# shg8/3DGS.cpp

Measured on NVIDIA B200. Metric: frames/sec, higher is better.
Workload: dtype f32

## Files before the change

### 3dgs.cpp_b200/csrc/gsb_api.cu

```cuda
#include <math.h>
#include <stdio.h>
#include <stdlib.h>
#include <string.h>

#include <algorithm>
#include <new>
#include <thread>
#include <vector>

#include "gsb_ctx.cuh"

using namespace gsb;

namespace {
thread_local std::string g_create_error;
}

namespace gsb {

int fail(gsb_ctx* c, int code, const char* what, cudaError_t e) {
    if (c) {
        c->err = what;
        if (e != cudaSuccess) {
            c->err += ": ";
// ... 108 lines not shown
    SortParams sa{};
    sa.keys[0] = ctx->dkeys[0];
    sa.keys[1] = ctx->dkeys[1];
    sa.vals[0] = ctx->dvals[0];
    sa.vals[1] = ctx->dvals[1];
    sa.key_bytes = 4;
    sa.d_m = &ctx->ctl->num_visible;
    sa.m_hint = fp.nv_q;
    sa.key_bits = 32;
    sa.status = ctx->sort_status;
    sa.status_tiles = ctx->sort_status_tiles;
    sa.d_epoch = &ctx->ctl->epoch;
    sa.epoch_base = 0;
    sa.sc = &ctx->ctl->sort_depth;
    sa.num_sms = ctx->num_sms;
    sa.events = nullptr;
    sa.ranges = nullptr;
    sa.discard_sorted_keys = true;
    uint32_t depth_passes = 0;
    CK(launch_sort(sa, &depth_passes, stream));
    const int fin_a = depth_passes & 1;
    if (events) CK(cudaEventRecord(ctx->ev[2], stream));

    EmitParams ep{};
    ep.sorted_cid = ctx->dvals[fin_a];
    ep.nv_hint = fp.nv_q;
    ep.tiles_x = fp.bins_x;
    ep.coarse_shift = fp.cs;
    ep.keys = ctx->keys[0];
    ep.vals = ctx->vals[0];
    ep.capacity = (uint32_t)ctx->capacity;
// ... 22 lines not shown
    SortParams sp{};
    sp.keys[0] = ctx->keys[0];
    sp.keys[1] = ctx->keys[1];
    sp.vals[0] = ctx->vals[0];
    sp.vals[1] = ctx->vals[1];
    sp.key_bytes = 4;
    sp.d_m = &ctx->ctl->num_instances;
    sp.m_hint = fp.m_q;
    sp.key_bits = bits_for(fp.bins);
    sp.status = ctx->sort_status;
    sp.status_tiles = ctx->sort_status_tiles;
    sp.d_epoch = &ctx->ctl->epoch;
    sp.epoch_base = 4;
    sp.sc = &ctx->ctl->sort_tile;
    sp.num_sms = ctx->num_sms;
    sp.events = events ? ctx->ev_sort : nullptr;
    sp.ranges = ctx->ranges;
    sp.discard_sorted_keys = !ctx->debug && fp.cs == 0;
    sp.range_key_mask = fp.cs ? 0xffffu : 0u;
    uint32_t passes = 0;
    CK(launch_sort(sp, &passes, stream));
    if (events) CK(cudaEventRecord(ctx->ev[4], stream));
    if (passes == 0) CK(launch_ranges_single_tile(sp.d_m, ctx->ranges, stream));
    if (events) CK(cudaEventRecord(ctx->ev[5], stream));
    if (depth_passes != fp.depth_passes || passes != fp.passes) return fail(ctx, GSB_ERR_CUDA, "internal: pass count mismatch");
    return GSB_OK;
}

int launch_middle_graph(gsb_ctx* ctx, const FramePlan& fp, cudaStream_t stream) {
    MiddleKey key;
    key.tiles_x = fp.tiles_x;
// ... 146 lines not shown
    bp.variant = ctx->blend_variant;
    bp.stats = ctx->debug ? 2 : (ctx->timers ? 1 : 0);
    bp.one = 1.0f;
    bp.ctl = ctx->ctl;
    if (band_aux) {
        bp.aux = reinterpret_cast<float2*>(static_cast<unsigned char*>(band_aux) + (size_t)(b0 - fp.rb) * GSB_TILE * aux_pitch);
        bp.aux_pitch = aux_pitch;
    }
    CK(launch_blend(bp, stream));
    return GSB_OK;
}

int enqueue_tail(gsb_ctx* ctx, const FramePlan& fp, cudaStream_t stream) {
    if (ctx->timers) CK(cudaEventRecord(ctx->ev[6], stream));
    CK(cudaMemcpyAsync(ctx->ctl_host, ctx->ctl, offsetof(Control, sort_depth), cudaMemcpyDeviceToHost, stream));
    CK(cudaEventRecord(ctx->ev_done, stream));
    ctx->frame_pending = true;
    ctx->have_frame = true;
    ctx->frame_debug = ctx->debug;
    ctx->frame_timers = ctx->timers;
    ctx->last_w = fp.W;
    ctx->last_h = fp.H;
    ctx->last_tiles_x = fp.tiles_x;
    ctx->last_tiles_y = fp.tiles_y;
    ctx->last_passes = fp.passes;
    ctx->last_depth_passes = fp.depth_passes;
    ctx->last_final = (uint32_t)fp.fin;
    return GSB_OK;
}

// ... 71 lines not shown
        gsb_destroy(ctx);
        return GSB_ERR_NO_DEVICE;
    }
    ctx->num_sms = prop.multiProcessorCount;
    if (const char* v = getenv("GSB_BLEND_VARIANT")) ctx->blend_variant = atoi(v) == 1 ? 1 : 2;
    if (const char* v = getenv("GSB_HOST_DIRECT")) ctx->host_direct = atoi(v) != 0;
    if (const char* v = getenv("GSB_COARSE_SHIFT")) ctx->coarse_shift = (uint32_t)std::min(2, std::max(1, atoi(v)));
    if ((e = sort_prepare()) != cudaSuccess) return bail("sort_prepare", e);
    if ((e = cudaStreamCreateWithFlags(&ctx->stream, cudaStreamNonBlocking)) != cudaSuccess) return bail("cudaStreamCreate", e);
    if ((e = dev_alloc(&ctx->ctl, 1)) != cudaSuccess) return bail("cudaMalloc", e);
    if ((e = cudaMemset(ctx->ctl, 0, sizeof(Control))) != cudaSuccess) return bail("cudaMemset", e);
    if ((e = cudaDeviceSynchronize()) != cudaSuccess) return bail("cudaDeviceSynchronize", e);
    if ((e = cudaMallocHost(reinterpret_cast<void**>(&ctx->ctl_host), sizeof(Control))) != cudaSuccess) return bail("cudaMallocHost", e);
    memset(ctx->ctl_host, 0, sizeof(Control));
    for (auto& ev : ctx->ev)
        if ((e = cudaEventCreate(&ev)) != cudaSuccess) return bail("cudaEventCreate", e);
    for (auto& ev : ctx->ev_sort)
        if ((e = cudaEventCreate(&ev)) != cudaSuccess) return bail("cudaEventCreate", e);
    if ((e = cudaEventCreateWithFlags(&ctx->ev_done, cudaEventDisableTiming)) != cudaSuccess) return bail("cudaEventCreate", e);
    *out = ctx;
    return GSB_OK;
}

void gsb_destroy(gsb_ctx* ctx) {
    if (!ctx) return;
    cudaSetDevice(ctx->device);
    if (ctx->stream) cudaStreamSynchronize(ctx->stream);
    cudaDeviceSynchronize();
    drop_graphs(ctx);
    shard_destroy(ctx);
    dev_free(ctx->dbg_offsets);
    dev_free(ctx->pos_op);
// ... 6 lines not shown
    dev_free(ctx->emit_status);
    dev_free(ctx->recs);
    dev_free(ctx->dkeys[0]);
    dev_free(ctx->dkeys[1]);
    dev_free(ctx->dvals[0]);
    dev_free(ctx->dvals[1]);
    free_arena(ctx);
    dev_free(ctx->ranges);
    if (ctx->fb) cudaFree(ctx->fb);
    if (ctx->aux_fb) cudaFree(ctx->aux_fb);
    dev_free(ctx->dbg_tiles);
    dev_free(ctx->dbg_aabb);
    dev_free(ctx->dbg_keys_unsorted);
    dev_free(ctx->dbg_vals_unsorted);
    for (auto& ev : ctx->ev)
        if (ev) cudaEventDestroy(ev);
    for (auto& ev : ctx->ev_sort)
        if (ev) cudaEventDestroy(ev);
    if (ctx->ev_done) cudaEventDestroy(ctx->ev_done);
    if (ctx->stream) cudaStreamDestroy(ctx->stream);
    delete ctx;
}

int gsb_scene_upload(gsb_ctx* ctx, const float* vertices, uint64_t n, gsb_memory mem) {
    if (!ctx) return GSB_ERR_INVALID;
    if (n && !vertices) return fail(ctx, GSB_ERR_INVALID, "null vertices");
    if (n >= (1ull << 30)) return fail(ctx, GSB_ERR_INVALID, "scene limited to 2^30 - 1 Gaussians");
    CK(cudaSetDevice(ctx->device));
    CK(cudaStreamSynchronize(ctx->stream));
    ctx->frame_pending = false;
    ctx->have_frame = false;
    dev_free(ctx->pos_op);
// ... 292 lines not shown
    out->sort_passes = ctx->last_passes;
    out->sort_depth_passes = ctx->last_depth_passes;
    out->regrow_count = ctx->regrow_count;
    if (ctx->frame_timers) {
        float ms = 0.f;
        CK(cudaEventElapsedTime(&ms, ctx->ev[0], ctx->ev[1]));
        out->preprocess_ms = ms;
        CK(cudaEventElapsedTime(&ms, ctx->ev[1], ctx->ev[2]));
        out->sort_depth_ms = ms;
        CK(cudaEventElapsedTime(&ms, ctx->ev[2], ctx->ev[3]));
        out->preprocess_sort_ms = ms;
        CK(cudaEventElapsedTime(&ms, ctx->ev[3], ctx->ev[4]));
        out->sort_tile_ms = ms;
        out->sort_ms = out->sort_depth_ms + out->sort_tile_ms;
        if (ctx->last_passes) {
            CK(cudaEventElapsedTime(&ms, ctx->ev[3], ctx->ev_sort[0]));
            out->sort_hist_ms = ms;
            for (uint32_t p = 0; p < ctx->last_passes && p < 8; p++) {
                CK(cudaEventElapsedTime(&ms, ctx->ev_sort[p], ctx->ev_sort[p + 1]));
                out->sort_pass_ms[p] = ms;
            }
        }
        CK(cudaEventElapsedTime(&ms, ctx->ev[4], ctx->ev[5]));
        out->tile_boundary_ms = ms;
        CK(cudaEventElapsedTime(&ms, ctx->ev[5], ctx->ev[6]));
        out->render_ms = ms;
        CK(cudaEventElapsedTime(&ms, ctx->ev[0], ctx->ev[6]));
        out->frame_ms = ms;
        if (ctx->shard) {
            CK(cudaEventElapsedTime(&ms, ctx->ev[5], ctx->ev[7]));
            out->shard_blend_ms = ms;
            CK(cudaEventElapsedTime(&ms, ctx->ev[7], ctx->ev[6]));
            out->shard_wait_ms = ms;
        }
    }
    if (c->overflow || c->overflow_sticky) {
// ... 179 lines not shown
    SortParams sp{};
    sp.keys[0] = keys;
    sp.keys[1] = keys_tmp;
    sp.key_bytes = key_bytes;
    sp.vals[0] = vals;
    sp.vals[1] = vals_tmp;
    sp.d_m = &ctx->ctl->num_instances;
    sp.m_hint = m32;
    sp.key_bits = key_bits;
    sp.status = status;
    sp.status_tiles = tiles;
    sp.d_epoch = nullptr;
    sp.epoch_base = 8;
    sp.sc = &ctx->ctl->sort_tile;
    sp.num_sms = ctx->num_sms;
    sp.events = nullptr;
    sp.ranges = nullptr;
    uint32_t passes = 0;
    if (e == cudaSuccess) e = launch_sort(sp, &passes, s);
    if (e == cudaSuccess && (passes & 1)) {
        e = cudaMemcpyAsync(keys, keys_tmp, m * (size_t)key_bytes, cudaMemcpyDeviceToDevice, s);
        if (e == cudaSuccess) e = cudaMemcpyAsync(vals, vals_tmp, m * 4, cudaMemcpyDeviceToDevice, s);
    }
    if (e == cudaSuccess) e = cudaStreamSynchronize(s);
    cudaFree(status);
    if (e != cudaSuccess) return fail(ctx, GSB_ERR_CUDA, what, e);
    return GSB_OK;
}

int gsb_sort_pairs(gsb_ctx* ctx, uint64_t* keys, uint32_t* vals, uint64_t* keys_tmp, uint32_t* vals_tmp, uint64_t m,
                   uint32_t key_bits, void* stream) {
// ... 10 lines not shown
```

### 3dgs.cpp_b200/csrc/gsb_ctx.cuh

```cuda
#pragma once
#include <algorithm>
#include <string>

#include "gsb_internal.cuh"

namespace gsb {
struct ShardState;
}
using gsb::Control;

struct MiddleKey {
    uint32_t tiles_x = 0, num_tiles = 0, nv_q = 0, m_q = 0, cull = 0, tag = 0, cs = 0;
    uint64_t alloc_gen = 0;
    bool operator==(const MiddleKey& o) const {
        return tiles_x == o.tiles_x && num_tiles == o.num_tiles && nv_q == o.nv_q && m_q == o.m_q && cull == o.cull && tag == o.tag &&
               cs == o.cs && alloc_gen == o.alloc_gen;
    }
};
struct MiddleGraph {
    MiddleKey key;
    cudaGraphExec_t exec = nullptr;
    uint64_t last_use = 0;
};

// ... 26 lines not shown
    uint32_t sort_status_tiles = 0;
    uint32_t epoch = 8;
    uint2* ranges = nullptr;
    uint32_t ranges_tiles = 0;
    void* fb = nullptr;
    size_t fb_bytes = 0;
    void* aux_fb = nullptr;
    size_t aux_fb_bytes = 0;

    int mode = GSB_MODE_EXACT;
    bool debug = false;
    bool timers = true;
    int tile_cull = 0;
    uint32_t coarse_shift = 2;
    cudaEvent_t ev[8] = {};
    cudaEvent_t ev_sort[9] = {};
    cudaEvent_t ev_done = nullptr;
    bool frame_pending = false;
    bool have_frame = false;
    bool frame_debug = false;
    bool frame_timers = false;
    bool host_direct = true;
    int blend_variant = 2;
    bool use_graph = true;
    uint64_t alloc_gen = 0;
    uint64_t graph_clock = 0;
    uint32_t frames_since_epoch_clear = 0;
    MiddleGraph graphs[4] = {};
    uint32_t m_hint = 0;
    uint32_t nv_hint = 0;
    uint32_t regrow_count = 0;
// ... 63 lines not shown
```

### 3dgs.cpp_b200/csrc/gsb_internal.cuh

```cuda
#pragma once
#include <cuda_runtime.h>
#include <stdint.h>

#include <string>

#include "gs_b200.h"

#define GSB_TILE 16
#define GSB_REC_F4 4
#define GSB_MAX_SHARDS 8

namespace gsb {

struct SortCtl {
    uint32_t ticket[8];
    uint32_t hist[8][256];
};

struct Control {
    uint32_t project_ticket;
    uint32_t emit_ticket;
    uint32_t num_visible;
    uint32_t num_instances;
    uint32_t overflow;
    uint32_t overflow_sticky;
    uint32_t epoch;
    uint32_t pad0;
    unsigned long long instances_total;
    unsigned long long blend_consumed;
    unsigned long long candidates_total;
// ... 52 lines not shown
cudaError_t launch_emit(const EmitParams& p, cudaStream_t s);

struct SortParams {
    void* keys[2];
    uint32_t* vals[2];
    int key_bytes;
    const uint32_t* d_m;
    uint32_t m_hint;
    uint32_t key_bits;
    unsigned long long* status;
    uint32_t status_tiles;
    const uint32_t* d_epoch;
    uint32_t epoch_base;
    SortCtl* sc;
    int num_sms;
    cudaEvent_t* events;
    uint2* ranges;
    uint32_t range_key_mask;
    bool discard_sorted_keys;
};
cudaError_t launch_sort(const SortParams& p, uint32_t* passes, cudaStream_t s);
uint32_t sort_tile_items();

cudaError_t launch_frame_init(Control* ctl, uint32_t* project_status, uint32_t project_chunks, unsigned long long* emit_status,
                              uint32_t emit_chunks, uint2* ranges, uint32_t num_tiles, cudaStream_t s, uint32_t* extra_words = nullptr,
                              uint32_t num_extra_words = 0);
cudaError_t sort_prepare();
cudaError_t launch_ranges_single_tile(const uint32_t* d_m, uint2* ranges, cudaStream_t s);

struct BlendParams {
    const float4* recs;
// ... 24 lines not shown
```

### 3dgs.cpp_b200/csrc/gsb_sort.cu

```cuda
#include "gsb_internal.cuh"
#include "gsb_tma.cuh"

namespace gsb {

namespace {

#ifndef GSB_SORT_MATCH_ATOMIC
#define GSB_SORT_MATCH_ATOMIC 1
#endif
constexpr int SORT_IPT = 16;
#ifndef GSB_SORT_THREADS
#define GSB_SORT_THREADS 256
#endif
constexpr int SORT_THREADS = GSB_SORT_THREADS;
constexpr int SORT_TILE = SORT_THREADS * SORT_IPT;
constexpr int SORT_WARPS = SORT_THREADS / 32;
constexpr int RADIX = 256;
constexpr unsigned FULL = 0xffffffffu;

#ifndef GSB_HIST_CTAS
#define GSB_HIST_CTAS 3
#endif
constexpr int HIST_THREADS = 512;
constexpr int HIST_IPT = 8;
constexpr int HIST_TILE = HIST_THREADS * HIST_IPT;

constexpr uint32_t LB_AGG = 1u << 30;
constexpr uint32_t LB_PREFIX = 2u << 30;
constexpr uint32_t LB_COUNT = (1u << 30) - 1u;
#ifndef GSB_LB_WINDOW
#define GSB_LB_WINDOW 8
#endif
constexpr int LB_WINDOW = GSB_LB_WINDOW;

__device__ __forceinline__ unsigned long long ld_volatile(const unsigned long long* p) {
    return *reinterpret_cast<const volatile unsigned long long*>(p);
}
__device__ __forceinline__ void st_volatile(unsigned long long* p, unsigned long long v) {
    *reinterpret_cast<volatile unsigned long long*>(p) = v;
}

template <typename KeyT>
__device__ __forceinline__ KeyT key_max();
template <>
__device__ __forceinline__ uint32_t key_max<uint32_t>() {
    return 0xffffffffu;
}
template <>
__device__ __forceinline__ unsigned long long key_max<unsigned long long>() {
    return ~0ull;
}

template <typename KeyT, int P>
__global__ void __launch_bounds__(HIST_THREADS) k_sort_hist(const KeyT* __restrict__ keys, const uint32_t* __restrict__ d_m,
                                                            SortCtl* sc) {
    __shared__ uint32_t s_hist[P][RADIX];
    const int tid = threadIdx.x;
    for (int k = tid; k < P * RADIX; k += HIST_THREADS) (&s_hist[0][0])[k] = 0;
    __syncthreads();
    const uint32_t m = *d_m;
    const uint32_t num_tiles = (m + HIST_TILE - 1) / HIST_TILE;
    for (uint32_t tile = blockIdx.x; tile < num_tiles; tile += gridDim.x) {
        const uint32_t base = tile * HIST_TILE;
        KeyT k[HIST_IPT];
#pragma unroll
        for (int it = 0; it < HIST_IPT; it++) {
            const uint32_t idx = base + it * HIST_THREADS + tid;
            k[it] = idx < m ? __ldg(keys + idx) : key_max<KeyT>();
        }
#pragma unroll
        for (int it = 0; it < HIST_IPT; it++) {
            const uint32_t idx = base + it * HIST_THREADS + tid;
            const bool valid = idx < m;
#pragma unroll
            for (int p = 0; p < P; p++) {
                const uint32_t d = (uint32_t)(k[it] >> (8 * p)) & 255u;
                const uint32_t d0 = __shfl_sync(FULL, d, 0);
                const unsigned same = __ballot_sync(FULL, valid && d == d0);
                if ((threadIdx.x & 31) == 0) {
                    if (same) atomicAdd(&s_hist[p][d0], (uint32_t)__popc(same));
                } else if (valid && d != d0) {
                    atomicAdd(&s_hist[p][d], 1u);
                }
            }
        }
    }
    __syncthreads();
    for (int k = tid; k < P * RADIX; k += HIST_THREADS) {
        const uint32_t c = (&s_hist[0][0])[k];
        if (c) atomicAdd(&sc->hist[0][0] + k, c);
    }
}

template <typename KeyT>
constexpr bool kMatchAtomic = GSB_SORT_MATCH_ATOMIC && sizeof(KeyT) == 4;
template <typename KeyT>
struct PassSmem {
    KeyT keys[2][SORT_TILE];
    uint32_t vals[2][SORT_TILE];
    uint32_t whist[SORT_WARPS][RADIX];
    uint32_t match[kMatchAtomic<KeyT> ? SORT_WARPS : 1][RADIX];
    uint32_t bin_start[RADIX];
    int32_t out_base[RADIX];
    uint32_t gexcl[RADIX];
    uint32_t warp_sums[SORT_WARPS];
    unsigned long long mbar[2];
// ... 27 lines not shown
        if (lane >= o) incl += t;
    }
    if (lane == 31) warp_sums[warp] = incl;
    __syncthreads();
    uint32_t before = 0;
#pragma unroll
    for (int w = 0; w < NW; w++) {
        const uint32_t s = warp_sums[w];
        if (w < warp) before += s;
    }
    __syncthreads();
    return before + incl - v;
}

template <typename KeyT>
__global__ void __launch_bounds__(SORT_THREADS, ctas_per_sm<KeyT>())
    k_onesweep_pass(const KeyT* __restrict__ kin, const uint32_t* __restrict__ vin, KeyT* __restrict__ kout,
                    uint32_t* __restrict__ vout, const uint32_t* __restrict__ d_m, SortCtl* sc, int pass,
                    unsigned long long* status, uint32_t status_tiles, const uint32_t* __restrict__ d_epoch, uint32_t epoch_off,
                    uint2* __restrict__ ranges, uint32_t range_mask) {
    extern __shared__ __align__(128) unsigned char smem_raw[];
    PassSmem<KeyT>& S = *reinterpret_cast<PassSmem<KeyT>*>(smem_raw);
    const int tid = threadIdx.x, lane = tid & 31, warp = tid >> 5;
    const int shift = 8 * pass;
    const uint32_t m = *d_m;
    uint32_t num_tiles = (m + SORT_TILE - 1) / SORT_TILE;
    if (num_tiles > status_tiles) num_tiles = status_tiles;
    const uint32_t epoch = (d_epoch ? *d_epoch : 0u) + epoch_off;
    const unsigned long long epoch_hi = (unsigned long long)epoch << 32;

    auto fetch = [&](int buf) {
        const uint32_t t = atomicAdd(&sc->ticket[pass], 1u);
        S.tile[buf] = t;
        if (t < num_tiles && m - t * SORT_TILE >= (uint32_t)SORT_TILE) {
            fence_proxy_async();
            mbar_expect_tx(&S.mbar[buf], SORT_TILE * (sizeof(KeyT) + 4));
            tma_load(S.keys[buf], kin + (size_t)t * SORT_TILE, SORT_TILE * sizeof(KeyT), &S.mbar[buf]);
            tma_load(S.vals[buf], vin + (size_t)t * SORT_TILE, SORT_TILE * 4, &S.mbar[buf]);
        }
    };

    if (tid == 0) {
        mbar_init(&S.mbar[0], 1);
        mbar_init(&S.mbar[1], 1);
        mbar_fence_init();
    }
    {
        const uint32_t c = tid < RADIX ? sc->hist[pass][tid] : 0u;
        const uint32_t ex = block_excl_scan<SORT_WARPS>(c, S.warp_sums);
        if (tid < RADIX) S.gexcl[tid] = ex;
    }
    if constexpr (kMatchAtomic<KeyT>)
        for (int k = tid; k < SORT_WARPS * RADIX; k += SORT_THREADS) (&S.match[0][0])[k] = 0u;
    if (tid == 0) fetch(0);
    __syncthreads();

    int cur = 0;
    uint32_t parity0 = 0u, parity1 = 0u;
    while (true) {
        const uint32_t tile = S.tile[cur];
        if (tile >= num_tiles) break;
        if (tid == 0) fetch(cur ^ 1);
        const uint32_t tile_base = tile * SORT_TILE;
        const uint32_t valid = min((uint32_t)SORT_TILE, m - tile_base);
        KeyT* sk = S.keys[cur];
        uint32_t* sv = S.vals[cur];

#pragma unroll
        for (int k = 0; k < SORT_WARPS * RADIX / SORT_THREADS; k++) (&S.whist[0][0])[k * SORT_THREADS + tid] = 0;
        if (valid == (uint32_t)SORT_TILE) {
            if (cur == 0) {
                mbar_wait(&S.mbar[0], parity0);
                parity0 ^= 1u;
            } else {
                mbar_wait(&S.mbar[1], parity1);
                parity1 ^= 1u;
            }
        } else {
#pragma unroll 4
            for (int it = 0; it < SORT_IPT; it++) {
                const uint32_t li = it * SORT_THREADS + tid;
                const bool ok = li < valid;
                sk[li] = ok ? __ldg(kin + tile_base + li) : key_max<KeyT>();
                sv[li] = ok ? __ldg(vin + tile_base + li) : 0u;
            }
        }
        __syncthreads();

        const uint32_t wbase = warp * (32 * SORT_IPT) + lane;
        uint16_t rank[SORT_IPT];
        {
            uint32_t dg[SORT_IPT];
#pragma unroll
            for (int it = 0; it < SORT_IPT; it++) dg[it] = sw((uint32_t)(sk[wbase + it * 32] >> shift) & 255u);
            if constexpr (kMatchAtomic<KeyT>) {
#pragma unroll
            for (int it = 0; it < SORT_IPT; it++) {
                volatile uint32_t* mm = &S.match[warp][dg[it]];
                atomicOr(const_cast<uint32_t*>(mm), 1u << lane);
                __syncwarp();
                const unsigned peers = *mm;
                __syncwarp();
                const int leader = __ffs(peers) - 1;
                uint32_t prev = 0;
                if (lane == leader) {
                    *mm = 0u;
                    prev = S.whist[warp][dg[it]];
                    S.whist[warp][dg[it]] = prev + __popc(peers);
                }
                prev = __shfl_sync(FULL, prev, leader);
                rank[it] = (uint16_t)(prev + __popc(peers & ((1u << lane) - 1u)));
                __syncwarp();
            }
            } else {
            unsigned peers[SORT_IPT];
#pragma unroll
            for (int it = 0; it < SORT_IPT; it++) peers[it] = match_digit8(dg[it]);
#pragma unroll
            for (int it = 0; it < SORT_IPT; it++) {
                const int leader = __ffs(peers[it]) - 1;
                uint32_t prev = 0;
                if (lane == leader) {
                    prev = S.whist[warp][dg[it]];
                    S.whist[warp][dg[it]] = prev + __popc(peers[it]);
                }
                prev = __shfl_sync(FULL, prev, leader);
                rank[it] = (uint16_t)(prev + __popc(peers[it] & ((1u << lane) - 1u)));
                __syncwarp();
            }
            }
        }
        __syncthreads();

        uint32_t count = 0;
        if (tid < RADIX) {
#pragma unroll
            for (int w = 0; w < SORT_WARPS; w++) {
                const uint32_t c = S.whist[w][sw(tid)];
                S.whist[w][sw(tid)] = count;
                count += c;
            }
            st_volatile(status + (size_t)tile * RADIX + tid, epoch_hi | (tile == 0 ? LB_PREFIX : LB_AGG) | count);
        }
        const uint32_t bstart = block_excl_scan<SORT_WARPS>(count, S.warp_sums);
        if (tid < RADIX) S.bin_start[sw(tid)] = bstart;
        __syncthreads();

        {
            KeyT key[SORT_IPT];
            uint32_t val[SORT_IPT];
            uint32_t pos[SORT_IPT];
#pragma unroll
            for (int it = 0; it < SORT_IPT; it++) {
                key[it] = sk[wbase + it * 32];
                val[it] = sv[wbase + it * 32];
            }
#pragma unroll
            for (int it = 0; it < SORT_IPT; it++) {
                const uint32_t d = sw((uint32_t)(key[it] >> shift) & 255u);
                pos[it] = S.bin_start[d] + S.whist[warp][d] + rank[it];
            }
            __syncthreads();
#pragma unroll
            for (int it = 0; it < SORT_IPT; it++) {
                sk[pos[it]] = key[it];
                sv[pos[it]] = val[it];
            }
        }

        if (tid < RADIX) {
            uint32_t excl = 0;
            int t = (int)tile - 1;
            bool done = tile == 0;
            while (!done) {
                unsigned long long w[LB_WINDOW];
#pragma unroll
                for (int j = 0; j < LB_WINDOW; j++)
                    w[j] = (t - j >= 0) ? ld_volatile(status + (size_t)(t - j) * RADIX + tid) : (epoch_hi | LB_PREFIX);
#pragma unroll
                for (int j = 0; j < LB_WINDOW; j++) {
                    if (done) break;
                    const uint32_t lo = (uint32_t)w[j];
                    if ((w[j] >> 32) != epoch) break;
                    excl += lo & LB_COUNT;
                    --t;
                    if (lo & LB_PREFIX) done = true;
                }
            }
            if (tile != 0) st_volatile(status + (size_t)tile * RADIX + tid, epoch_hi | LB_PREFIX | (excl + count));
            S.out_base[sw(tid)] = (int32_t)(S.gexcl[tid] + excl) - (int32_t)bstart;
        }
        __syncthreads();

        {
            KeyT k[SORT_IPT];
            uint32_t v[SORT_IPT];
            int32_t g[SORT_IPT];
#pragma unroll
            for (int it = 0; it < SORT_IPT; it++) {
                k[it] = sk[it * SORT_THREADS + tid];
                v[it] = sv[it * SORT_THREADS + tid];
            }
#pragma unroll
            for (int it = 0; it < SORT_IPT; it++)
                g[it] = S.out_base[sw((uint32_t)(k[it] >> shift) & 255u)] + (int32_t)(it * SORT_THREADS + tid);
#pragma unroll
            for (int it = 0; it < SORT_IPT; it++) {
                if ((uint32_t)(it * SORT_THREADS + tid) < valid) {
                    if (kout != nullptr) kout[g[it]] = k[it];
                    vout[g[it]] = v[it];
                }
            }
            if (ranges != nullptr) {
                if constexpr (sizeof(KeyT) == 4) {
#pragma unroll
                    for (int it = 0; it < SORT_IPT; it++) {
                        const uint32_t idx = (uint32_t)(it * SORT_THREADS + tid);
                        if (idx < valid) {
                            const uint32_t key = (uint32_t)k[it] & range_mask;
                            if (idx == 0 || ((uint32_t)sk[idx - 1] & range_mask) != key) atomicMin(&ranges[key].x, (uint32_t)g[it]);
                            if (idx == valid - 1 || ((uint32_t)sk[idx + 1] & range_mask) != key) atomicMin(&ranges[key].y, ~((uint32_t)g[it] + 1u));
                        }
                    }
                }
            }
        }
        __syncthreads();
        cur ^= 1;
    }
}

template <typename KeyT>
cudaError_t launch_hist(const KeyT* keys, const SortParams& p, uint32_t P, uint32_t blocks, cudaStream_t s) {
    switch (P) {
        case 1: k_sort_hist<KeyT, 1><<<blocks, HIST_THREADS, 0, s>>>(keys, p.d_m, p.sc); break;
        case 2: k_sort_hist<KeyT, 2><<<blocks, HIST_THREADS, 0, s>>>(keys, p.d_m, p.sc); break;
        case 3: k_sort_hist<KeyT, 3><<<blocks, HIST_THREADS, 0, s>>>(keys, p.d_m, p.sc); break;
        case 4: k_sort_hist<KeyT, 4><<<blocks, HIST_THREADS, 0, s>>>(keys, p.d_m, p.sc); break;
        default:
            if constexpr (sizeof(KeyT) == 8) {
                switch (P) {
                    case 5: k_sort_hist<KeyT, 5><<<blocks, HIST_THREADS, 0, s>>>(keys, p.d_m, p.sc); break;
                    case 6: k_sort_hist<KeyT, 6><<<blocks, HIST_THREADS, 0, s>>>(keys, p.d_m, p.sc); break;
                    case 7: k_sort_hist<KeyT, 7><<<blocks, HIST_THREADS, 0, s>>>(keys, p.d_m, p.sc); break;
                    default: k_sort_hist<KeyT, 8><<<blocks, HIST_THREADS, 0, s>>>(keys, p.d_m, p.sc); break;
                }
            } else {
                return cudaErrorInvalidValue;
            }
    }
    return cudaGetLastError();
}

template <typename KeyT>
cudaError_t launch_sort_t(const SortParams& p, uint32_t P, cudaStream_t s) {
    const uint32_t hint = p.m_hint ? p.m_hint : 1;
    KeyT* keys[2] = {static_cast<KeyT*>(p.keys[0]), static_cast<KeyT*>(p.keys[1])};
    {
        uint32_t blocks = (hint + HIST_TILE - 1) / HIST_TILE;
        const uint32_t cap = (uint32_t)p.num_sms * GSB_HIST_CTAS;
        if (blocks > cap) blocks = cap;
        if (blocks == 0) blocks = 1;
        cudaError_t e = launch_hist<KeyT>(keys[0], p, P, blocks, s);
        if (e != cudaSuccess) return e;
        if (p.events && (e = cudaEventRecord(p.events[0], s)) != cudaSuccess) return e;
    }
    const size_t smem = sizeof(PassSmem<KeyT>);
    uint32_t blocks = (hint + SORT_TILE - 1) / SORT_TILE;
    const uint32_t cap = (uint32_t)p.num_sms * ctas_per_sm<KeyT>();
    if (blocks > cap) blocks = cap;
    if (blocks == 0) blocks = 1;
    for (uint32_t pass = 0; pass < P; pass++) {
        const int src = pass & 1, dst = src ^ 1;
        KeyT* kout = (pass + 1 == P && p.discard_sorted_keys) ? nullptr : keys[dst];
        k_onesweep_pass<KeyT><<<blocks, SORT_THREADS, smem, s>>>(keys[src], p.vals[src], kout, p.vals[dst], p.d_m, p.sc,
                                                                 (int)pass, p.status, p.status_tiles, p.d_epoch, p.epoch_base + pass,
                                                                 pass + 1 == P ? p.ranges : nullptr, p.range_key_mask ? p.range_key_mask : 0xffffffffu);
        cudaError_t e = cudaGetLastError();
        if (e != cudaSuccess) return e;
        if (p.events && (e = cudaEventRecord(p.events[1 + pass], s)) != cudaSuccess) return e;
    }
    return cudaSuccess;
}

}

uint32_t sort_tile_items() { return SORT_TILE; }

cudaError_t sort_prepare() {
    cudaError_t e = cudaFuncSetAttribute(k_onesweep_pass<uint32_t>, cudaFuncAttributeMaxDynamicSharedMemorySize,
                                         (int)sizeof(PassSmem<uint32_t>));
    if (e != cudaSuccess) return e;
    return cudaFuncSetAttribute(k_onesweep_pass<unsigned long long>, cudaFuncAttributeMaxDynamicSharedMemorySize,
                                (int)sizeof(PassSmem<unsigned long long>));
}

cudaError_t launch_sort(const SortParams& p, uint32_t* passes, cudaStream_t s) {
    const uint32_t P = (p.key_bits + 7) / 8;
    *passes = P;
    if (P == 0) return cudaSuccess;
    if (p.key_bytes == 4 && P <= 4) return launch_sort_t<uint32_t>(p, P, s);
    if (p.key_bytes == 8 && P <= 8) return launch_sort_t<unsigned long long>(p, P, s);
    return cudaErrorInvalidValue;
}

namespace {
__global__ void k_ranges_single_tile(const uint32_t* __restrict__ d_m, uint2* __restrict__ ranges) {
    const uint32_t m = *d_m;
// ... 11 lines not shown
```

Baseline: 827.9.

## Fuse radix sort histogram and all onesweep passes into one persistent kernel

Replaces the separate histogram kernel and per-pass onesweep launches with a single persistent kernel. It computes the histograms with dynamic tile tickets, then runs every pass, separated by software grid barriers built on acquire/release atomics. Per-pass CUDA events give way to globaltimer stamps stored in the control block. This removes multiple kernel launches and their tail drains per sort. In exchange it relies on every CTA being co-resident for the spin barriers, and the histogram phase now runs at the sort kernel's occupancy.

```diff
diff --git a/3dgs.cpp_b200/csrc/gsb_api.cu b/3dgs.cpp_b200/csrc/gsb_api.cu
--- a/3dgs.cpp_b200/csrc/gsb_api.cu
+++ b/3dgs.cpp_b200/csrc/gsb_api.cu
@@ -146,7 +146,6 @@
     sa.epoch_base = 0;
     sa.sc = &ctx->ctl->sort_depth;
     sa.num_sms = ctx->num_sms;
-    sa.events = nullptr;
     sa.ranges = nullptr;
     sa.discard_sorted_keys = true;
     uint32_t depth_passes = 0;
@@ -199,7 +198,6 @@
     sp.epoch_base = 4;
     sp.sc = &ctx->ctl->sort_tile;
     sp.num_sms = ctx->num_sms;
-    sp.events = events ? ctx->ev_sort : nullptr;
     sp.ranges = ctx->ranges;
     sp.discard_sorted_keys = !ctx->debug && fp.cs == 0;
     sp.range_key_mask = fp.cs ? 0xffffu : 0u;
@@ -376,6 +374,9 @@
 int enqueue_tail(gsb_ctx* ctx, const FramePlan& fp, cudaStream_t stream) {
     if (ctx->timers) CK(cudaEventRecord(ctx->ev[6], stream));
     CK(cudaMemcpyAsync(ctx->ctl_host, ctx->ctl, offsetof(Control, sort_depth), cudaMemcpyDeviceToHost, stream));
+    if (ctx->timers)
+        CK(cudaMemcpyAsync(ctx->ctl_host->sort_tile.stamp, ctx->ctl->sort_tile.stamp, sizeof(ctx->ctl->sort_tile.stamp),
+                           cudaMemcpyDeviceToHost, stream));
     CK(cudaEventRecord(ctx->ev_done, stream));
     ctx->frame_pending = true;
     ctx->have_frame = true;
@@ -477,8 +478,6 @@
     if ((e = cudaMallocHost(reinterpret_cast<void**>(&ctx->ctl_host), sizeof(Control))) != cudaSuccess) return bail("cudaMallocHost", e);
     memset(ctx->ctl_host, 0, sizeof(Control));
     for (auto& ev : ctx->ev)
-        if ((e = cudaEventCreate(&ev)) != cudaSuccess) return bail("cudaEventCreate", e);
-    for (auto& ev : ctx->ev_sort)
         if ((e = cudaEventCreate(&ev)) != cudaSuccess) return bail("cudaEventCreate", e);
     if ((e = cudaEventCreateWithFlags(&ctx->ev_done, cudaEventDisableTiming)) != cudaSuccess) return bail("cudaEventCreate", e);
     *out = ctx;
@@ -515,8 +514,6 @@
     dev_free(ctx->dbg_keys_unsorted);
     dev_free(ctx->dbg_vals_unsorted);
     for (auto& ev : ctx->ev)
-        if (ev) cudaEventDestroy(ev);
-    for (auto& ev : ctx->ev_sort)
         if (ev) cudaEventDestroy(ev);
     if (ctx->ev_done) cudaEventDestroy(ctx->ev_done);
     if (ctx->stream) cudaStreamDestroy(ctx->stream);
@@ -839,12 +836,9 @@
         out->sort_tile_ms = ms;
         out->sort_ms = out->sort_depth_ms + out->sort_tile_ms;
         if (ctx->last_passes) {
-            CK(cudaEventElapsedTime(&ms, ctx->ev[3], ctx->ev_sort[0]));
-            out->sort_hist_ms = ms;
-            for (uint32_t p = 0; p < ctx->last_passes && p < 8; p++) {
-                CK(cudaEventElapsedTime(&ms, ctx->ev_sort[p], ctx->ev_sort[p + 1]));
-                out->sort_pass_ms[p] = ms;
-            }
+            const unsigned long long* t = c->sort_tile.stamp;
+            out->sort_hist_ms = (float)(t[1] - t[0]) * 1e-6f;
+            for (uint32_t p = 0; p < ctx->last_passes && p < 8; p++) out->sort_pass_ms[p] = (float)(t[2 + p] - t[1 + p]) * 1e-6f;
         }
         CK(cudaEventElapsedTime(&ms, ctx->ev[4], ctx->ev[5]));
         out->tile_boundary_ms = ms;
@@ -1054,7 +1048,6 @@
     sp.epoch_base = 8;
     sp.sc = &ctx->ctl->sort_tile;
     sp.num_sms = ctx->num_sms;
-    sp.events = nullptr;
     sp.ranges = nullptr;
     uint32_t passes = 0;
     if (e == cudaSuccess) e = launch_sort(sp, &passes, s);
diff --git a/3dgs.cpp_b200/csrc/gsb_ctx.cuh b/3dgs.cpp_b200/csrc/gsb_ctx.cuh
--- a/3dgs.cpp_b200/csrc/gsb_ctx.cuh
+++ b/3dgs.cpp_b200/csrc/gsb_ctx.cuh
@@ -64,7 +64,6 @@
     int tile_cull = 0;
     uint32_t coarse_shift = 2;
     cudaEvent_t ev[8] = {};
-    cudaEvent_t ev_sort[9] = {};
     cudaEvent_t ev_done = nullptr;
     bool frame_pending = false;
     bool have_frame = false;
diff --git a/3dgs.cpp_b200/csrc/gsb_internal.cuh b/3dgs.cpp_b200/csrc/gsb_internal.cuh
--- a/3dgs.cpp_b200/csrc/gsb_internal.cuh
+++ b/3dgs.cpp_b200/csrc/gsb_internal.cuh
@@ -14,6 +14,11 @@
 
 struct SortCtl {
     uint32_t ticket[8];
+    uint32_t done[8];
+    uint32_t hist_ticket;
+    uint32_t hist_done;
+    uint32_t pad[2];
+    unsigned long long stamp[10];
     uint32_t hist[8][256];
 };
 
@@ -96,7 +101,7 @@
     uint32_t epoch_base;
     SortCtl* sc;
     int num_sms;
-    cudaEvent_t* events;
+    bool hist_ready;
     uint2* ranges;
     uint32_t range_key_mask;
     bool discard_sorted_keys;
diff --git a/3dgs.cpp_b200/csrc/gsb_sort.cu b/3dgs.cpp_b200/csrc/gsb_sort.cu
--- a/3dgs.cpp_b200/csrc/gsb_sort.cu
+++ b/3dgs.cpp_b200/csrc/gsb_sort.cu
@@ -18,13 +18,6 @@
 constexpr int RADIX = 256;
 constexpr unsigned FULL = 0xffffffffu;
 
-#ifndef GSB_HIST_CTAS
-#define GSB_HIST_CTAS 3
-#endif
-constexpr int HIST_THREADS = 512;
-constexpr int HIST_IPT = 8;
-constexpr int HIST_TILE = HIST_THREADS * HIST_IPT;
-
 constexpr uint32_t LB_AGG = 1u << 30;
 constexpr uint32_t LB_PREFIX = 2u << 30;
 constexpr uint32_t LB_COUNT = (1u << 30) - 1u;
@@ -39,6 +32,22 @@
 __device__ __forceinline__ void st_volatile(unsigned long long* p, unsigned long long v) {
     *reinterpret_cast<volatile unsigned long long*>(p) = v;
 }
+__device__ __forceinline__ uint32_t ld_acquire(const uint32_t* p) {
+    uint32_t v;
+    asm volatile("ld.acquire.gpu.global.u32 %0, [%1];" : "=r"(v) : "l"(p) : "memory");
+    return v;
+}
+__device__ __forceinline__ uint32_t atomic_add_acq_rel(uint32_t* p, uint32_t v) {
+    uint32_t old;
+    asm volatile("atom.acq_rel.gpu.global.add.u32 %0, [%1], %2;" : "=r"(old) : "l"(p), "r"(v) : "memory");
+    return old;
+}
+__device__ __forceinline__ unsigned long long global_timer() {
+    unsigned long long t;
+    asm volatile("mov.u64 %0, %%globaltimer;" : "=l"(t));
+    return t;
+}
+__device__ __forceinline__ void fence_proxy_async_global() { asm volatile("fence.proxy.async.global;" ::: "memory"); }
 
 template <typename KeyT>
 __device__ __forceinline__ KeyT key_max();
@@ -49,47 +58,6 @@
 template <>
 __device__ __forceinline__ unsigned long long key_max<unsigned long long>() {
     return ~0ull;
-}
-
-template <typename KeyT, int P>
-__global__ void __launch_bounds__(HIST_THREADS) k_sort_hist(const KeyT* __restrict__ keys, const uint32_t* __restrict__ d_m,
-                                                            SortCtl* sc) {
-    __shared__ uint32_t s_hist[P][RADIX];
-    const int tid = threadIdx.x;
-    for (int k = tid; k < P * RADIX; k += HIST_THREADS) (&s_hist[0][0])[k] = 0;
-    __syncthreads();
-    const uint32_t m = *d_m;
-    const uint32_t num_tiles = (m + HIST_TILE - 1) / HIST_TILE;
-    for (uint32_t tile = blockIdx.x; tile < num_tiles; tile += gridDim.x) {
-        const uint32_t base = tile * HIST_TILE;
-        KeyT k[HIST_IPT];
-#pragma unroll
-        for (int it = 0; it < HIST_IPT; it++) {
-            const uint32_t idx = base + it * HIST_THREADS + tid;
-            k[it] = idx < m ? __ldg(keys + idx) : key_max<KeyT>();
-        }
-#pragma unroll
-        for (int it = 0; it < HIST_IPT; it++) {
-            const uint32_t idx = base + it * HIST_THREADS + tid;
-            const bool valid = idx < m;
-#pragma unroll
-            for (int p = 0; p < P; p++) {
-                const uint32_t d = (uint32_t)(k[it] >> (8 * p)) & 255u;
-                const uint32_t d0 = __shfl_sync(FULL, d, 0);
-                const unsigned same = __ballot_sync(FULL, valid && d == d0);
-                if ((threadIdx.x & 31) == 0) {
-                    if (same) atomicAdd(&s_hist[p][d0], (uint32_t)__popc(same));
-                } else if (valid && d != d0) {
-                    atomicAdd(&s_hist[p][d], 1u);
-                }
-            }
-        }
-    }
-    __syncthreads();
-    for (int k = tid; k < P * RADIX; k += HIST_THREADS) {
-        const uint32_t c = (&s_hist[0][0])[k];
-        if (c) atomicAdd(&sc->hist[0][0] + k, c);
-    }
 }
 
 template <typename KeyT>
@@ -147,273 +115,347 @@
 }
 
 template <typename KeyT>
-__global__ void __launch_bounds__(SORT_THREADS, ctas_per_sm<KeyT>())
-    k_onesweep_pass(const KeyT* __restrict__ kin, const uint32_t* __restrict__ vin, KeyT* __restrict__ kout,
-                    uint32_t* __restrict__ vout, const uint32_t* __restrict__ d_m, SortCtl* sc, int pass,
-                    unsigned long long* status, uint32_t status_tiles, const uint32_t* __restrict__ d_epoch, uint32_t epoch_off,
-                    uint2* __restrict__ ranges, uint32_t range_mask) {
+__device__ __forceinline__ uint32_t hist_phase(PassSmem<KeyT>& S, const KeyT* kin, uint32_t m, int P, SortCtl* sc) {
+    const int tid = threadIdx.x, lane = tid & 31, warp = tid >> 5;
+    uint32_t* h = &S.whist[0][0];
+    static_assert(SORT_WARPS * RADIX >= 8 * RADIX, "whist holds the histograms of up to 8 passes");
+    for (int k = tid; k < P * RADIX; k += SORT_THREADS) h[k] = 0u;
+    const uint32_t num_tiles = (m + SORT_TILE - 1) / SORT_TILE;
+    uint32_t mine = 0;
+    while (true) {
+        if (tid == 0) S.tile[0] = atomicAdd(&sc->hist_ticket, 1u);
+        __syncthreads();
+        const uint32_t tile = S.tile[0];
+        __syncthreads();
+        if (tile >= num_tiles) break;
+        mine++;
+        const uint32_t base = tile * SORT_TILE;
+        KeyT k[SORT_IPT];
+#pragma unroll
+        for (int it = 0; it < SORT_IPT; it++) {
+            const uint32_t idx = base + it * SORT_THREADS + tid;
+            k[it] = idx < m ? __ldcg(kin + idx) : key_max<KeyT>();
+        }
+#pragma unroll
+        for (int it = 0; it < SORT_IPT; it++) {
+            const unsigned valid = __ballot_sync(FULL, base + it * SORT_THREADS + tid < m);
+            for (int p = 0; p < P; p++) {
+                const uint32_t d = (uint32_t)(k[it] >> (8 * p)) & 255u;
+                unsigned peers;
+                if constexpr (kMatchAtomic<KeyT>) {
+                    volatile uint32_t* mm = &S.match[warp][d];
+                    atomicOr(const_cast<uint32_t*>(mm), 1u << lane);
+                    __syncwarp();
+                    peers = *mm;
+                    __syncwarp();
+                } else {
+                    peers = match_digit8(d);
+                }
+                if (lane == __ffs(peers) - 1) {
+                    if constexpr (kMatchAtomic<KeyT>) *const_cast<volatile uint32_t*>(&S.match[warp][d]) = 0u;
+                    const uint32_t c = __popc(peers & valid);
+                    if (c) atomicAdd(&h[p * RADIX + d], c);
+                }
+                __syncwarp();
+            }
+        }
+    }
+    for (int k = tid; k < P * RADIX; k += SORT_THREADS) {
+        const uint32_t c = h[k];
+        if (c) atomicAdd(&sc->hist[0][0] + k, c);
+    }
+    return mine;
+}
+
+__device__ __forceinline__ void grid_barrier(uint32_t* done, uint32_t mine, uint32_t total, unsigned long long* stamp) {
+    __syncthreads();
+    if (threadIdx.x == 0) {
+        const bool last = mine != 0 ? atomic_add_acq_rel(done, mine) + mine == total : (total == 0 && blockIdx.x == 0);
+        if (last) *stamp = global_timer();
+        while (ld_acquire(done) < total) {
+        }
+        fence_proxy_async_global();
+    }
+    __syncthreads();
+}
+
+template <typename KeyT>
+struct SortArgs {
+    KeyT* keys[2];
+    uint32_t* vals[2];
+    const uint32_t* d_m;
+    SortCtl* sc;
+    unsigned long long* status;
+    uint32_t status_tiles;
+    const uint32_t* d_epoch;
+    uint32_t epoch_base;
+    uint2* ranges;
+    uint32_t range_mask;
+    int passes;
+    int hist_phase;
+    int discard_last_keys;
+};
+
+template <typename KeyT>
+__global__ void __launch_bounds__(SORT_THREADS, ctas_per_sm<KeyT>()) k_onesweep(const __grid_constant__ SortArgs<KeyT> A) {
     extern __shared__ __align__(128) unsigned char smem_raw[];
     PassSmem<KeyT>& S = *reinterpret_cast<PassSmem<KeyT>*>(smem_raw);
     const int tid = threadIdx.x, lane = tid & 31, warp = tid >> 5;
-    const int shift = 8 * pass;
-    const uint32_t m = *d_m;
+    SortCtl* sc = A.sc;
+    unsigned long long* status = A.status;
+    if (tid == 0 && blockIdx.x == 0) sc->stamp[0] = global_timer();
+    const uint32_t m = *A.d_m;
     uint32_t num_tiles = (m + SORT_TILE - 1) / SORT_TILE;
-    if (num_tiles > status_tiles) num_tiles = status_tiles;
-    const uint32_t epoch = (d_epoch ? *d_epoch : 0u) + epoch_off;
-    const unsigned long long epoch_hi = (unsigned long long)epoch << 32;
-
-    auto fetch = [&](int buf) {
-        const uint32_t t = atomicAdd(&sc->ticket[pass], 1u);
-        S.tile[buf] = t;
-        if (t < num_tiles && m - t * SORT_TILE >= (uint32_t)SORT_TILE) {
-            fence_proxy_async();
-            mbar_expect_tx(&S.mbar[buf], SORT_TILE * (sizeof(KeyT) + 4));
-            tma_load(S.keys[buf], kin + (size_t)t * SORT_TILE, SORT_TILE * sizeof(KeyT), &S.mbar[buf]);
-            tma_load(S.vals[buf], vin + (size_t)t * SORT_TILE, SORT_TILE * 4, &S.mbar[buf]);
-        }
-    };
+    if (num_tiles > A.status_tiles) num_tiles = A.status_tiles;
+    const uint32_t epoch0 = (A.d_epoch ? *A.d_epoch : 0u) + A.epoch_base;
 
     if (tid == 0) {
         mbar_init(&S.mbar[0], 1);
         mbar_init(&S.mbar[1], 1);
         mbar_fence_init();
     }
-    {
-        const uint32_t c = tid < RADIX ? sc->hist[pass][tid] : 0u;
-        const uint32_t ex = block_excl_scan<SORT_WARPS>(c, S.warp_sums);
-        if (tid < RADIX) S.gexcl[tid] = ex;
-    }
     if constexpr (kMatchAtomic<KeyT>)
         for (int k = tid; k < SORT_WARPS * RADIX; k += SORT_THREADS) (&S.match[0][0])[k] = 0u;
-    if (tid == 0) fetch(0);
     __syncthreads();
+    if (A.hist_phase) {
+        const uint32_t mine = hist_phase<KeyT>(S, A.keys[0], m, A.passes, sc);
+        grid_barrier(&sc->hist_done, mine, (m + SORT_TILE - 1) / SORT_TILE, &sc->stamp[1]);
+    } else if (tid == 0 && blockIdx.x == 0) {
+        sc->stamp[1] = sc->stamp[0];
+    }
 
     int cur = 0;
     uint32_t parity0 = 0u, parity1 = 0u;
-    while (true) {
-        const uint32_t tile = S.tile[cur];
-        if (tile >= num_tiles) break;
-        if (tid == 0) fetch(cur ^ 1);
-        const uint32_t tile_base = tile * SORT_TILE;
-        const uint32_t valid = min((uint32_t)SORT_TILE, m - tile_base);
-        KeyT* sk = S.keys[cur];
-        uint32_t* sv = S.vals[cur];
-
-#pragma unroll
-        for (int k = 0; k < SORT_WARPS * RADIX / SORT_THREADS; k++) (&S.whist[0][0])[k * SORT_THREADS + tid] = 0;
-        if (valid == (uint32_t)SORT_TILE) {
-            if (cur == 0) {
-                mbar_wait(&S.mbar[0], parity0);
-                parity0 ^= 1u;
+    for (int pass = 0; pass < A.passes; pass++) {
+        const int shift = 8 * pass;
+        const KeyT* kin = A.keys[pass & 1];
+        const uint32_t* vin = A.vals[pass & 1];
+        KeyT* kout = (pass + 1 == A.passes && A.discard_last_keys) ? nullptr : A.keys[(pass & 1) ^ 1];
+        uint32_t* vout = A.vals[(pass & 1) ^ 1];
+        uint2* ranges = pass + 1 == A.passes ? A.ranges : nullptr;
+        const uint32_t range_mask = A.range_mask;
+        const uint32_t epoch = epoch0 + pass;
+        const unsigned long long epoch_hi = (unsigned long long)epoch << 32;
+
+        auto fetch = [&](int buf) {
+            const uint32_t t = atomicAdd(&sc->ticket[pass], 1u);
+            S.tile[buf] = t;
+            if (t < num_tiles && m - t * SORT_TILE >= (uint32_t)SORT_TILE) {
+                fence_proxy_async();
+                mbar_expect_tx(&S.mbar[buf], SORT_TILE * (sizeof(KeyT) + 4));
+                tma_load(S.keys[buf], kin + (size_t)t * SORT_TILE, SORT_TILE * sizeof(KeyT), &S.mbar[buf]);
+                tma_load(S.vals[buf], vin + (size_t)t * SORT_TILE, SORT_TILE * 4, &S.mbar[buf]);
+            }
+        };
+
+        if (tid == 0) fetch(cur);
+        {
+            const uint32_t c = tid < RADIX ? __ldcg(&sc->hist[pass][tid]) : 0u;
+            const uint32_t ex = block_excl_scan<SORT_WARPS>(c, S.warp_sums);
+            if (tid < RADIX) S.gexcl[tid] = ex;
+        }
+        uint32_t mine = 0;
+        while (true) {
+            const uint32_t tile = S.tile[cur];
+            if (tile >= num_tiles) break;
+            mine++;
+            if (tid == 0) fetch(cur ^ 1);
+            const uint32_t tile_base = tile * SORT_TILE;
+            const uint32_t valid = min((uint32_t)SORT_TILE, m - tile_base);
+            KeyT* sk = S.keys[cur];
+            uint32_t* sv = S.vals[cur];
+
+#pragma unroll
+            for (int k = 0; k < SORT_WARPS * RADIX / SORT_THREADS; k++) (&S.whist[0][0])[k * SORT_THREADS + tid] = 0;
+            if (valid == (uint32_t)SORT_TILE) {
+                if (cur == 0) {
+                    mbar_wait(&S.mbar[0], parity0);
+                    parity0 ^= 1u;
+                } else {
+                    mbar_wait(&S.mbar[1], parity1);
+                    parity1 ^= 1u;
+                }
             } else {
-                mbar_wait(&S.mbar[1], parity1);
-                parity1 ^= 1u;
-            }
-        } else {
 #pragma unroll 4
-            for (int it = 0; it < SORT_IPT; it++) {
-                const uint32_t li = it * SORT_THREADS + tid;
-                const bool ok = li < valid;
-                sk[li] = ok ? __ldg(kin + tile_base + li) : key_max<KeyT>();
-                sv[li] = ok ? __ldg(vin + tile_base + li) : 0u;
-            }
-        }
-        __syncthreads();
-
-        const uint32_t wbase = warp * (32 * SORT_IPT) + lane;
-        uint16_t rank[SORT_IPT];
-        {
-            uint32_t dg[SORT_IPT];
-#pragma unroll
-            for (int it = 0; it < SORT_IPT; it++) dg[it] = sw((uint32_t)(sk[wbase + it * 32] >> shift) & 255u);
-            if constexpr (kMatchAtomic<KeyT>) {
-#pragma unroll
-            for (int it = 0; it < SORT_IPT; it++) {
-                volatile uint32_t* mm = &S.match[warp][dg[it]];
-                atomicOr(const_cast<uint32_t*>(mm), 1u << lane);
-                __syncwarp();
-                const unsigned peers = *mm;
-                __syncwarp();
-                const int leader = __ffs(peers) - 1;
-                uint32_t prev = 0;
-                if (lane == leader) {
-                    *mm = 0u;
-                    prev = S.whist[warp][dg[it]];
-                    S.whist[warp][dg[it]] = prev + __popc(peers);
-                }
-                prev = __shfl_sync(FULL, prev, leader);
-                rank[it] = (uint16_t)(prev + __popc(peers & ((1u << lane) - 1u)));
-                __syncwarp();
-            }
-            } else {
-            unsigned peers[SORT_IPT];
-#pragma unroll
-            for (int it = 0; it < SORT_IPT; it++) peers[it] = match_digit8(dg[it]);
-#pragma unroll
-            for (int it = 0; it < SORT_IPT; it++) {
-                const int leader = __ffs(peers[it]) - 1;
-                uint32_t prev = 0;
-                if (lane == leader) {
-                    prev = S.whist[warp][dg[it]];
-                    S.whist[warp][dg[it]] = prev + __popc(peers[it]);
-                }
-                prev = __shfl_sync(FULL, prev, leader);
-                rank[it] = (uint16_t)(prev + __popc(peers[it] & ((1u << lane) - 1u)));
-                __syncwarp();
-            }
-            }
-        }
-        __syncthreads();
-
-        uint32_t count = 0;
-        if (tid < RADIX) {
-#pragma unroll
-            for (int w = 0; w < SORT_WARPS; w++) {
-                const uint32_t c = S.whist[w][sw(tid)];
-                S.whist[w][sw(tid)] = count;
-                count += c;
-            }
-            st_volatile(status + (size_t)tile * RADIX + tid, epoch_hi | (tile == 0 ? LB_PREFIX : LB_AGG) | count);
-        }
-        const uint32_t bstart = block_excl_scan<SORT_WARPS>(count, S.warp_sums);
-        if (tid < RADIX) S.bin_start[sw(tid)] = bstart;
-        __syncthreads();
-
-        {
-            KeyT key[SORT_IPT];
-            uint32_t val[SORT_IPT];
-            uint32_t pos[SORT_IPT];
-#pragma unroll
-            for (int it = 0; it < SORT_IPT; it++) {
-                key[it] = sk[wbase + it * 32];
-                val[it] = sv[wbase + it * 32];
-            }
-#pragma unroll
-            for (int it = 0; it < SORT_IPT; it++) {
-                const uint32_t d = sw((uint32_t)(key[it] >> shift) & 255u);
-                pos[it] = S.bin_start[d] + S.whist[warp][d] + rank[it];
+                for (int it = 0; it < SORT_IPT; it++) {
+                    const uint32_t li = it * SORT_THREADS + tid;
+                    const bool ok = li < valid;
+                    sk[li] = ok ? __ldcg(kin + tile_base + li) : key_max<KeyT>();
+                    sv[li] = ok ? __ldcg(vin + tile_base + li) : 0u;
+                }
             }
             __syncthreads();
-#pragma unroll
-            for (int it = 0; it < SORT_IPT; it++) {
-                sk[pos[it]] = key[it];
-                sv[pos[it]] = val[it];
-            }
-        }
-
-        if (tid < RADIX) {
-            uint32_t excl = 0;
-            int t = (int)tile - 1;
-            bool done = tile == 0;
-            while (!done) {
-                unsigned long long w[LB_WINDOW];
-#pragma unroll
-                for (int j = 0; j < LB_WINDOW; j++)
-                    w[j] = (t - j >= 0) ? ld_volatile(status + (size_t)(t - j) * RADIX + tid) : (epoch_hi | LB_PREFIX);
-#pragma unroll
-                for (int j = 0; j < LB_WINDOW; j++) {
-                    if (done) break;
-                    const uint32_t lo = (uint32_t)w[j];
-                    if ((w[j] >> 32) != epoch) break;
-                    excl += lo & LB_COUNT;
-                    --t;
-                    if (lo & LB_PREFIX) done = true;
-                }
-            }
-            if (tile != 0) st_volatile(status + (size_t)tile * RADIX + tid, epoch_hi | LB_PREFIX | (excl + count));
-            S.out_base[sw(tid)] = (int32_t)(S.gexcl[tid] + excl) - (int32_t)bstart;
-        }
-        __syncthreads();
-
-        {
-            KeyT k[SORT_IPT];
-            uint32_t v[SORT_IPT];
-            int32_t g[SORT_IPT];
-#pragma unroll
-            for (int it = 0; it < SORT_IPT; it++) {
-                k[it] = sk[it * SORT_THREADS + tid];
-                v[it] = sv[it * SORT_THREADS + tid];
-            }
-#pragma unroll
-            for (int it = 0; it < SORT_IPT; it++)
-                g[it] = S.out_base[sw((uint32_t)(k[it] >> shift) & 255u)] + (int32_t)(it * SORT_THREADS + tid);
-#pragma unroll
-            for (int it = 0; it < SORT_IPT; it++) {
-                if ((uint32_t)(it * SORT_THREADS + tid) < valid) {
-                    if (kout != nullptr) kout[g[it]] = k[it];
-                    vout[g[it]] = v[it];
-                }
-            }
-            if (ranges != nullptr) {
-                if constexpr (sizeof(KeyT) == 4) {
-#pragma unroll
-                    for (int it = 0; it < SORT_IPT; it++) {
-                        const uint32_t idx = (uint32_t)(it * SORT_THREADS + tid);
-                        if (idx < valid) {
-                            const uint32_t key = (uint32_t)k[it] & range_mask;
-                            if (idx == 0 || ((uint32_t)sk[idx - 1] & range_mask) != key) atomicMin(&ranges[key].x, (uint32_t)g[it]);
-                            if (idx == valid - 1 || ((uint32_t)sk[idx + 1] & range_mask) != key) atomicMin(&ranges[key].y, ~((uint32_t)g[it] + 1u));
+            const uint32_t wbase = warp * (32 * SORT_IPT) + lane;
+            uint16_t rank[SORT_IPT];
+            {
+                uint32_t dg[SORT_IPT];
+#pragma unroll
+                for (int it = 0; it < SORT_IPT; it++) dg[it] = sw((uint32_t)(sk[wbase + it * 32] >> shift) & 255u);
+                if constexpr (kMatchAtomic<KeyT>) {
+#pragma unroll
+                for (int it = 0; it < SORT_IPT; it++) {
+                    volatile uint32_t* mm = &S.match[warp][dg[it]];
+                    atomicOr(const_cast<uint32_t*>(mm), 1u << lane);
+                    __syncwarp();
+                    const unsigned peers = *mm;
+                    __syncwarp();
+                    const int leader = __ffs(peers) - 1;
+                    uint32_t prev = 0;
+                    if (lane == leader) {
+                        *mm = 0u;
+                        prev = S.whist[warp][dg[it]];
+                        S.whist[warp][dg[it]] = prev + __popc(peers);
+                    }
+                    prev = __shfl_sync(FULL, prev, leader);
+                    rank[it] = (uint16_t)(prev + __popc(peers & ((1u << lane) - 1u)));
+                    __syncwarp();
+                }
+                } else {
+                unsigned peers[SORT_IPT];
+#pragma unroll
+                for (int it = 0; it < SORT_IPT; it++) peers[it] = match_digit8(dg[it]);
+#pragma unroll
+                for (int it = 0; it < SORT_IPT; it++) {
+                    const int leader = __ffs(peers[it]) - 1;
+                    uint32_t prev = 0;
+                    if (lane == leader) {
+                        prev = S.whist[warp][dg[it]];
+                        S.whist[warp][dg[it]] = prev + __popc(peers[it]);
+                    }
+                    prev = __shfl_sync(FULL, prev, leader);
+                    rank[it] = (uint16_t)(prev + __popc(peers[it] & ((1u << lane) - 1u)));
+                    __syncwarp();
+                }
+                }
+            }
+            __syncthreads();
+
+            uint32_t count = 0;
+            if (tid < RADIX) {
+#pragma unroll
+                for (int w = 0; w < SORT_WARPS; w++) {
+                    const uint32_t c = S.whist[w][sw(tid)];
+                    S.whist[w][sw(tid)] = count;
+                    count += c;
+                }
+                st_volatile(status + (size_t)tile * RADIX + tid, epoch_hi | (tile == 0 ? LB_PREFIX : LB_AGG) | count);
+            }
+            const uint32_t bstart = block_excl_scan<SORT_WARPS>(count, S.warp_sums);
+            if (tid < RADIX) S.bin_start[sw(tid)] = bstart;
+            __syncthreads();
+
+            {
+                KeyT key[SORT_IPT];
+                uint32_t val[SORT_IPT];
+                uint32_t pos[SORT_IPT];
+#pragma unroll
+                for (int it = 0; it < SORT_IPT; it++) {
+                    key[it] = sk[wbase + it * 32];
+                    val[it] = sv[wbase + it * 32];
+                }
+#pragma unroll
+                for (int it = 0; it < SORT_IPT; it++) {
+                    const uint32_t d = sw((uint32_t)(key[it] >> shift) & 255u);
+                    pos[it] = S.bin_start[d] + S.whist[warp][d] + rank[it];
+                }
+                __syncthreads();
+#pragma unroll
+                for (int it = 0; it < SORT_IPT; it++) {
+                    sk[pos[it]] = key[it];
+                    sv[pos[it]] = val[it];
+                }
+            }
+
+            if (tid < RADIX) {
+                uint32_t excl = 0;
+                int t = (int)tile - 1;
+                bool done = tile == 0;
+                while (!done) {
+                    unsigned long long w[LB_WINDOW];
+#pragma unroll
+                    for (int j = 0; j < LB_WINDOW; j++)
+                        w[j] = (t - j >= 0) ? ld_volatile(status + (size_t)(t - j) * RADIX + tid) : (epoch_hi | LB_PREFIX);
+#pragma unroll
+                    for (int j = 0; j < LB_WINDOW; j++) {
+                        if (done) break;
+                        const uint32_t lo = (uint32_t)w[j];
+                        if ((w[j] >> 32) != epoch) break;
+                        excl += lo & LB_COUNT;
+                        --t;
+                        if (lo & LB_PREFIX) done = true;
+                    }
+                }
+                if (tile != 0) st_volatile(status + (size_t)tile * RADIX + tid, epoch_hi | LB_PREFIX | (excl + count));
+                S.out_base[sw(tid)] = (int32_t)(S.gexcl[tid] + excl) - (int32_t)bstart;
+            }
+            __syncthreads();
+
+            {
+                KeyT k[SORT_IPT];
+                uint32_t v[SORT_IPT];
+                int32_t g[SORT_IPT];
+#pragma unroll
+                for (int it = 0; it < SORT_IPT; it++) {
+                    k[it] = sk[it * SORT_THREADS + tid];
+                    v[it] = sv[it * SORT_THREADS + tid];
+                }
+#pragma unroll
+                for (int it = 0; it < SORT_IPT; it++)
+                    g[it] = S.out_base[sw((uint32_t)(k[it] >> shift) & 255u)] + (int32_t)(it * SORT_THREADS + tid);
+#pragma unroll
+                for (int it = 0; it < SORT_IPT; it++) {
+                    if ((uint32_t)(it * SORT_THREADS + tid) < valid) {
+                        if (kout != nullptr) kout[g[it]] = k[it];
+                        vout[g[it]] = v[it];
+                    }
+                }
+                if (ranges != nullptr) {
+                    if constexpr (sizeof(KeyT) == 4) {
+#pragma unroll
+                        for (int it = 0; it < SORT_IPT; it++) {
+                            const uint32_t idx = (uint32_t)(it * SORT_THREADS + tid);
+                            if (idx < valid) {
+                                const uint32_t key = (uint32_t)k[it] & range_mask;
+                                if (idx == 0 || ((uint32_t)sk[idx - 1] & range_mask) != key) atomicMin(&ranges[key].x, (uint32_t)g[it]);
+                                if (idx == valid - 1 || ((uint32_t)sk[idx + 1] & range_mask) != key) atomicMin(&ranges[key].y, ~((uint32_t)g[it] + 1u));
+                            }
                         }
                     }
                 }
             }
+            __syncthreads();
+            cur ^= 1;
         }
-        __syncthreads();
-        cur ^= 1;
-    }
-}
-
-template <typename KeyT>
-cudaError_t launch_hist(const KeyT* keys, const SortParams& p, uint32_t P, uint32_t blocks, cudaStream_t s) {
-    switch (P) {
-        case 1: k_sort_hist<KeyT, 1><<<blocks, HIST_THREADS, 0, s>>>(keys, p.d_m, p.sc); break;
-        case 2: k_sort_hist<KeyT, 2><<<blocks, HIST_THREADS, 0, s>>>(keys, p.d_m, p.sc); break;
-        case 3: k_sort_hist<KeyT, 3><<<blocks, HIST_THREADS, 0, s>>>(keys, p.d_m, p.sc); break;
-        case 4: k_sort_hist<KeyT, 4><<<blocks, HIST_THREADS, 0, s>>>(keys, p.d_m, p.sc); break;
-        default:
-            if constexpr (sizeof(KeyT) == 8) {
-                switch (P) {
-                    case 5: k_sort_hist<KeyT, 5><<<blocks, HIST_THREADS, 0, s>>>(keys, p.d_m, p.sc); break;
-                    case 6: k_sort_hist<KeyT, 6><<<blocks, HIST_THREADS, 0, s>>>(keys, p.d_m, p.sc); break;
-                    case 7: k_sort_hist<KeyT, 7><<<blocks, HIST_THREADS, 0, s>>>(keys, p.d_m, p.sc); break;
-                    default: k_sort_hist<KeyT, 8><<<blocks, HIST_THREADS, 0, s>>>(keys, p.d_m, p.sc); break;
-                }
-            } else {
-                return cudaErrorInvalidValue;
-            }
-    }
-    return cudaGetLastError();
+        grid_barrier(&sc->done[pass], mine, num_tiles, &sc->stamp[2 + pass]);
+    }
 }
 
 template <typename KeyT>
 cudaError_t launch_sort_t(const SortParams& p, uint32_t P, cudaStream_t s) {
     const uint32_t hint = p.m_hint ? p.m_hint : 1;
-    KeyT* keys[2] = {static_cast<KeyT*>(p.keys[0]), static_cast<KeyT*>(p.keys[1])};
-    {
-        uint32_t blocks = (hint + HIST_TILE - 1) / HIST_TILE;
-        const uint32_t cap = (uint32_t)p.num_sms * GSB_HIST_CTAS;
-        if (blocks > cap) blocks = cap;
-        if (blocks == 0) blocks = 1;
-        cudaError_t e = launch_hist<KeyT>(keys[0], p, P, blocks, s);
-        if (e != cudaSuccess) return e;
-        if (p.events && (e = cudaEventRecord(p.events[0], s)) != cudaSuccess) return e;
-    }
+    SortArgs<KeyT> a{};
+    a.keys[0] = static_cast<KeyT*>(p.keys[0]);
+    a.keys[1] = static_cast<KeyT*>(p.keys[1]);
+    a.vals[0] = p.vals[0];
+    a.vals[1] = p.vals[1];
+    a.d_m = p.d_m;
+    a.sc = p.sc;
+    a.status = p.status;
+    a.status_tiles = p.status_tiles;
+    a.d_epoch = p.d_epoch;
+    a.epoch_base = p.epoch_base;
+    a.ranges = p.ranges;
+    a.range_mask = p.range_key_mask ? p.range_key_mask : 0xffffffffu;
+    a.passes = (int)P;
+    a.hist_phase = p.hist_ready ? 0 : 1;
+    a.discard_last_keys = p.discard_sorted_keys ? 1 : 0;
     const size_t smem = sizeof(PassSmem<KeyT>);
     uint32_t blocks = (hint + SORT_TILE - 1) / SORT_TILE;
     const uint32_t cap = (uint32_t)p.num_sms * ctas_per_sm<KeyT>();
     if (blocks > cap) blocks = cap;
     if (blocks == 0) blocks = 1;
-    for (uint32_t pass = 0; pass < P; pass++) {
-        const int src = pass & 1, dst = src ^ 1;
-        KeyT* kout = (pass + 1 == P && p.discard_sorted_keys) ? nullptr : keys[dst];
-        k_onesweep_pass<KeyT><<<blocks, SORT_THREADS, smem, s>>>(keys[src], p.vals[src], kout, p.vals[dst], p.d_m, p.sc,
-                                                                 (int)pass, p.status, p.status_tiles, p.d_epoch, p.epoch_base + pass,
-                                                                 pass + 1 == P ? p.ranges : nullptr, p.range_key_mask ? p.range_key_mask : 0xffffffffu);
-        cudaError_t e = cudaGetLastError();
-        if (e != cudaSuccess) return e;
-        if (p.events && (e = cudaEventRecord(p.events[1 + pass], s)) != cudaSuccess) return e;
-    }
-    return cudaSuccess;
+    k_onesweep<KeyT><<<blocks, SORT_THREADS, smem, s>>>(a);
+    return cudaGetLastError();
 }
 
 }
@@ -421,10 +463,10 @@
 uint32_t sort_tile_items() { return SORT_TILE; }
 
 cudaError_t sort_prepare() {
-    cudaError_t e = cudaFuncSetAttribute(k_onesweep_pass<uint32_t>, cudaFuncAttributeMaxDynamicSharedMemorySize,
+    cudaError_t e = cudaFuncSetAttribute(k_onesweep<uint32_t>, cudaFuncAttributeMaxDynamicSharedMemorySize,
                                          (int)sizeof(PassSmem<uint32_t>));
     if (e != cudaSuccess) return e;
-    return cudaFuncSetAttribute(k_onesweep_pass<unsigned long long>, cudaFuncAttributeMaxDynamicSharedMemorySize,
+    return cudaFuncSetAttribute(k_onesweep<unsigned long long>, cudaFuncAttributeMaxDynamicSharedMemorySize,
                                 (int)sizeof(PassSmem<unsigned long long>));
 }
 
```

Result: slower. 806.0, median of 6 (-2.7%).
